# shinshoji01/Style-Restricted_GAN

Measured on AMD Instinct MI355X. Metric: images/sec G+D+E train step, CelebA 128x128 bs=32/GPU, higher is better.
Workload: dtype f32; 1 GPU; SRGAN-nopretrain (03-train) G+D+E train step, 128x128, bs=32/GPU, k=5, fp32, E trainable (BASELINE configs[1]); global_batch=32, unrolled_k=5, parallelism=dp1, graph_fallback=False, graph_segments=1, ranks_seen=1, execution=hipGraph replay of the captured step

## Files before the change

### style-restricted_gan_amd/csrc/conv_wino.hip

```cpp
#include <algorithm>
#include <cstdlib>
#include <type_traits>
#include "common.h"
#include "pack_device.h"

#ifndef WINO_EXP
#define WINO_EXP 0
#endif

namespace srgan {

constexpr int WT = 64;
constexpr int WNB = 64;
constexpr int WC = 8;

__device__ __forceinline__ auto uniform_rsrc(const float* base, unsigned bytes) {
  const unsigned long long a = reinterpret_cast<unsigned long long>(base);
  const unsigned lo = __builtin_amdgcn_readfirstlane((unsigned)a), hi = __builtin_amdgcn_readfirstlane((unsigned)(a >> 32));
  float* q = reinterpret_cast<float*>(((unsigned long long)hi << 32) | lo);
  return __builtin_amdgcn_make_buffer_rsrc(q, 0, __builtin_amdgcn_readfirstlane(bytes), 0x00020000);
}



template <int MODE, bool MASK = false>
__global__ __launch_bounds__(512) void wino_kernel(WinoParams p) {
  static_assert(!MASK || MODE == 2, "the mask epilogue exists for the transposed form only");
  constexpr int VH = 64 * 4 + 16, VP = 2 * VH + 32, VSZ = 16 * VP;
  static_assert(2 * VSZ <= 32768, "V buffers must fit the epilogue image");
  __shared__ __attribute__((aligned(16))) float lds[32768];
  __shared__ int tile_o[WT];
  __shared__ int tile_f[WT];
  constexpr int OT = MODE == 0 ? 2 : 3;
  constexpr int PS = MODE == 2 ? 2 : 1;
  const int ph_r = MODE == 2 ? (int)blockIdx.y >> 1 : 0, ph_s = MODE == 2 ? (int)blockIdx.y & 1 : 0;

  const int tid = threadIdx.x, lane = tid & 63, wave = tid >> 6;
  const int lr = lane & 31, lh = lane >> 5;
  int bid = blockIdx.x;
  const int nblk = gridDim.x;
  if ((nblk & 7) == 0) bid = (bid & 7) * (nblk >> 3) + (bid >> 3);
  const int m_tile = bid / p.n_tiles, n_tile = bid - m_tile * p.n_tiles;

  const int tl = tid >> 3, ch = tid & 7;
  constexpr unsigned kOutside = 0x80000000u;
  unsigned off[16];
  int g_b, g_ty, g_tx;
  bool g_tv;
  {
    const int t = m_tile * WT + tl;
    g_tv = t < p.T;
    const int tt = g_tv ? t : 0;
    const int per = p.TH * p.TW;
    g_b = tt / per;
    const int r = tt - g_b * per;
    g_ty = r / p.TW; g_tx = r - g_ty * p.TW;
    if (ch == 0) {
      const int oy = PS * OT * g_ty + ph_r, ox = PS * OT * g_tx + ph_s;
      const int nr = min(OT, (p.Ho - oy + PS - 1) / PS), nc = min(OT, (p.Wo - ox + PS - 1) / PS);
      tile_o[tl] = (g_tv && nr > 0 && nc > 0) ? (g_b * p.Ho + oy) * p.Wo + ox : -1;
      tile_f[tl] = max(nr, 0) | (max(nc, 0) << 4);
    }
  }
  auto set_offsets = [&](int phase) __attribute__((always_inline)) {
    int sy, dy_, oy0, ox0;
    if (MODE == 0) { sy = 2; dy_ = 1; oy0 = -p.pad; ox0 = -p.pad; }
    else if (MODE == 1) { sy = 6; dy_ = 2; oy0 = (phase >> 1) - p.pad; ox0 = (phase & 1) - p.pad; }
    else { sy = 3; dy_ = 1; oy0 = ph_r - 1; ox0 = ph_s - 1; }
#pragma unroll
    for (int i = 0; i < 4; ++i) {
      int iy = sy * g_ty + dy_ * i + oy0;
      bool yok = g_tv;
      if (MODE == 0 && p.reflect) {
        iy = iy < 0 ? -iy : iy;
        iy = iy >= p.H ? 2 * p.H - 2 - iy : iy;
        iy = min(max(iy, 0), p.H - 1);
      } else {
        yok = yok && (unsigned)iy < (unsigned)p.H;
      }
#pragma unroll
      for (int j = 0; j < 4; ++j) {
        int ix = sy * g_tx + dy_ * j + ox0;
        bool ok = yok;
        if (MODE == 0 && p.reflect) {
          ix = ix < 0 ? -ix : ix;
          ix = ix >= p.W ? 2 * p.W - 2 - ix : ix;
          ix = min(max(ix, 0), p.W - 1);
        } else {
          ok = ok && (unsigned)ix < (unsigned)p.W;
        }
        off[i * 4 + j] = ok ? (unsigned)(((g_b * p.H + iy) * p.W + ix) * p.C + ch) * 4u : kOutside;
      }
    }
  };
  set_offsets(0);
  const unsigned src_bytes = (unsigned)((size_t)p.NB * p.H * p.W * p.C * 4);
  const auto rs_x = uniform_rsrc(p.src, src_bytes);
  const auto rs_u = uniform_rsrc(p.u + ((size_t)(MODE == 2 ? blockIdx.y : 0) * p.n_tiles + n_tile) * p.nchunk * 8192,
                                 (unsigned)p.nchunk * 32768u);
  const unsigned ubase = (unsigned)((2 * wave) * 512 + lh * 256 + lr * 4) * 4u;

  float d[16];
  f32x4 bfr[2][2][2];
  int lc8 = 0, lphase = 0;
  auto load_x_part = [&](auto part_c) __attribute__((always_inline)) {
    constexpr int PART = decltype(part_c)::value;
#if WINO_EXP == 5 || WINO_EXP == 6
    if (lc8 + lphase > 0) return;
#endif
#pragma unroll
    for (int i = 4 * PART; i < 4 * PART + 4; ++i)
      d[i] = __builtin_bit_cast(float, __builtin_amdgcn_raw_buffer_load_b32(rs_x, off[i], lc8 * (WC * 4), 0));
    if constexpr (PART == 3) {
      ++lc8;
      if (MODE == 1 && lc8 == p.cpp) {
        lc8 = 0;
        ++lphase;
        set_offsets(lphase);
      }
    }
  };
  auto load_x = [&]() __attribute__((always_inline)) {
    load_x_part(std::integral_constant<int, 0>{});
    load_x_part(std::integral_constant<int, 1>{});
    load_x_part(std::integral_constant<int, 2>{});
    load_x_part(std::integral_constant<int, 3>{});
  };
  auto load_u1 = [&](int kc, auto par, int a, int j) __attribute__((always_inline)) {
    constexpr int P = decltype(par)::value;
#if WINO_EXP == 7
    if (kc > 1) return;
#endif
    bfr[P][a][j] = __builtin_bit_cast(f32x4, __builtin_amdgcn_raw_buffer_load_b128(rs_u, ubase + a * 2048 + j * 512, kc * 32768, 0));
  };
  auto load_u = [&](int kc, auto par) __attribute__((always_inline)) {
#pragma unroll
    for (int a = 0; a < 2; ++a)
#pragma unroll
      for (int j = 0; j < 2; ++j) load_u1(kc, par, a, j);
  };
  float tv[16];
  auto store_piece = [&](int buf, auto piece_c) __attribute__((always_inline)) {
    constexpr int PIECE = decltype(piece_c)::value;
#if WINO_EXP == 4 || WINO_EXP == 6
    return;
#endif
    float* V = lds + buf * VSZ + (ch >> 2) * VH + tl * 4 + (ch & 3);
    if constexpr (PIECE == 0) {
#if WINO_EXP == 9
      return;
#endif
#pragma unroll
      for (int c = 0; c < 4; ++c) {
        tv[0 * 4 + c] = d[0 * 4 + c] - d[2 * 4 + c];
        tv[1 * 4 + c] = d[1 * 4 + c] + d[2 * 4 + c];
        tv[2 * 4 + c] = d[2 * 4 + c] - d[1 * 4 + c];
        tv[3 * 4 + c] = d[1 * 4 + c] - d[3 * 4 + c];
      }
    } else {
#if WINO_EXP == 8
#pragma unroll
      for (int r = 2 * (PIECE - 1); r < 2 * PIECE; ++r) {
        asm volatile("" ::"v"(tv[r * 4 + 0] - tv[r * 4 + 2]), "v"(tv[r * 4 + 1] + tv[r * 4 + 2]), "v"(tv[r * 4 + 2] - tv[r * 4 + 1]),
                     "v"(tv[r * 4 + 1] - tv[r * 4 + 3]));
      }
      (void)V;
#elif WINO_EXP == 9
#pragma unroll
      for (int r = 2 * (PIECE - 1); r < 2 * PIECE; ++r) {
        V[(r * 4 + 0) * VP] = d[r * 4 + 0];
        V[(r * 4 + 1) * VP] = d[r * 4 + 1];
        V[(r * 4 + 2) * VP] = d[r * 4 + 2];
        V[(r * 4 + 3) * VP] = d[r * 4 + 3];
      }
#else
#pragma unroll
      for (int r = 2 * (PIECE - 1); r < 2 * PIECE; ++r) {
        V[(r * 4 + 0) * VP] = tv[r * 4 + 0] - tv[r * 4 + 2];
        V[(r * 4 + 1) * VP] = tv[r * 4 + 1] + tv[r * 4 + 2];
        V[(r * 4 + 2) * VP] = tv[r * 4 + 2] - tv[r * 4 + 1];
        V[(r * 4 + 3) * VP] = tv[r * 4 + 1] - tv[r * 4 + 3];
      }
#endif
    }
  };
  auto store_v = [&](int buf) __attribute__((always_inline)) {
    store_piece(buf, std::integral_constant<int, 0>{});
    store_piece(buf, std::integral_constant<int, 1>{});
    store_piece(buf, std::integral_constant<int, 2>{});
  };

  f32x16 acc[2][2][2];
#pragma unroll
  for (int a = 0; a < 2; ++a)
#pragma unroll
    for (int i = 0; i < 2; ++i)
#pragma unroll
      for (int j = 0; j < 2; ++j)
#pragma unroll
        for (int e = 0; e < 16; ++e) acc[a][i][j][e] = 0.f;

  f32x4 af[2][2];
  auto read_frags = [&](int buf, int slot) __attribute__((always_inline)) {
    const float* V = lds + buf * VSZ + (2 * wave + slot) * VP + lh * VH;
#pragma unroll
    for (int i = 0; i < 2; ++i) af[slot][i] = *reinterpret_cast<const f32x4*>(V + (i * 32 + lr) * 4);
  };
  auto mfma_steps = [&](auto par, int slot, int e0, int e1) __attribute__((always_inline)) {
    constexpr int P = decltype(par)::value;
#pragma unroll
    for (int e = e0; e < e1; ++e)
#pragma unroll
      for (int i = 0; i < 2; ++i)
#pragma unroll
        for (int j = 0; j < 2; ++j)
          acc[slot][i][j] = __builtin_amdgcn_mfma_f32_32x32x2f32(af[slot][i][e], bfr[P][slot][j][e], acc[slot][i][j], 0, 0, 0);
  };

  using I0 = std::integral_constant<int, 0>;
  using I1 = std::integral_constant<int, 1>;
  using I2 = std::integral_constant<int, 2>;
  using I3 = std::integral_constant<int, 3>;
  using T = std::true_type;
  using F = std::false_type;
  const int nk = p.nchunk;
  load_x();
  load_u(0, I0{});
  store_v(0);
  __syncthreads();
  read_frags(0, 0);
  if (nk > 1) load_x();
  auto iter = [&](int kc, auto par, auto st, auto ld) __attribute__((always_inline)) {
    constexpr bool ST = decltype(st)::value, LD = decltype(ld)::value;
    constexpr int P = decltype(par)::value;
    using NP = std::integral_constant<int, 1 - P>;
    auto sb = [&]() __attribute__((always_inline)) { __builtin_amdgcn_sched_barrier(0); };
    read_frags(P, 1);
    mfma_steps(par, 0, 0, 1);
    if constexpr (ST) store_piece(1 - P, I0{});
    sb();
    mfma_steps(par, 0, 1, 2);
    if constexpr (ST) store_piece(1 - P, I1{});
    if constexpr (LD) load_x_part(I0{});
    sb();
    mfma_steps(par, 0, 2, 3);
    if constexpr (ST) store_piece(1 - P, I2{});
    if constexpr (LD) load_x_part(I1{});
    sb();
    mfma_steps(par, 0, 3, 4);
    if constexpr (ST) load_u1(kc + 1, NP{}, 0, 0);
    if constexpr (LD) load_x_part(I2{});
    sb();
    mfma_steps(par, 1, 0, 1);
    if constexpr (ST) load_u1(kc + 1, NP{}, 0, 1);
    if constexpr (LD) load_x_part(I3{});
    sb();
    mfma_steps(par, 1, 1, 2);
    if constexpr (ST) { load_u1(kc + 1, NP{}, 1, 0); load_u1(kc + 1, NP{}, 1, 1); }
    sb();
    mfma_steps(par, 1, 2, 3);
    sb();
    __syncthreads();
    if constexpr (ST) read_frags(1 - P, 0);
    mfma_steps(par, 1, 3, 4);
  };
  {
    int kc = 0;
    for (; kc + 3 < nk; kc += 2) {
      iter(kc, I0{}, T{}, T{});
      iter(kc + 1, I1{}, T{}, T{});
    }
    iter(kc, I0{}, T{}, F{});
    iter(kc + 1, I1{}, F{}, F{});
  }

  const int cq = tid & 7, et = tid >> 3;
#pragma unroll
  for (int half = 0; half < 2; ++half) {
    __syncthreads();
#pragma unroll
    for (int a = 0; a < 2; ++a)
#pragma unroll
      for (int i = 0; i < 2; ++i)
#pragma unroll
        for (int e = 0; e < 16; ++e) {
          const int tile = i * 32 + (e & 3) + 8 * (e >> 2) + 4 * lh;
          lds[(2 * wave + a) * 2048 + tile * 32 + lr] = acc[a][i][half][e];
        }
    __syncthreads();
    const int n = n_tile * WNB + half * 32 + cq * 4;
    const bool nok = n < p.Cd;
    f32x4 bv = {0.f, 0.f, 0.f, 0.f};
    if (nok && p.bias) bv = *reinterpret_cast<const f32x4*>(p.bias + n);
    const int o = tile_o[et], f = tile_f[et];
    f32x4 mk[OT][OT];
    if constexpr (MASK) {
      if (nok && o >= 0) {
        const float* mp = p.mask + (size_t)o * p.Cd + n;
#pragma unroll
        for (int a = 0; a < OT; ++a)
#pragma unroll
          for (int b2 = 0; b2 < OT; ++b2)
            if (a < (f & 15) && b2 < (f >> 4)) mk[a][b2] = *reinterpret_cast<const f32x4*>(mp + (size_t)(a * p.Wo + b2) * PS * p.Cd);
      }
    }
    f32x4 m[16];
#pragma unroll
    for (int k = 0; k < 16; ++k) m[k] = *reinterpret_cast<const f32x4*>(lds + k * 2048 + et * 32 + cq * 4);
    f32x4 y[OT][OT];
    if constexpr (MODE == 0) {
      f32x4 s0[4], s1[4];
#pragma unroll
      for (int c = 0; c < 4; ++c) {
        s0[c] = m[0 * 4 + c] + m[1 * 4 + c] + m[2 * 4 + c];
        s1[c] = m[1 * 4 + c] - m[2 * 4 + c] - m[3 * 4 + c];
      }
      y[0][0] = s0[0] + s0[1] + s0[2]; y[0][1] = s0[1] - s0[2] - s0[3];
      y[1][0] = s1[0] + s1[1] + s1[2]; y[1][1] = s1[1] - s1[2] - s1[3];
    } else {
      f32x4 h[3][4];
#pragma unroll
      for (int c = 0; c < 4; ++c) {
        h[0][c] = m[0 * 4 + c] + 0.5f * (m[1 * 4 + c] + m[2 * 4 + c]);
        h[1][c] = 0.5f * (m[1 * 4 + c] - m[2 * 4 + c]);
        h[2][c] = 0.5f * (m[1 * 4 + c] + m[2 * 4 + c]) + m[3 * 4 + c];
      }
#pragma unroll
      for (int a = 0; a < 3; ++a) {
        y[a][0] = h[a][0] + 0.5f * (h[a][1] + h[a][2]);
        y[a][1] = 0.5f * (h[a][1] - h[a][2]);
        y[a][2] = 0.5f * (h[a][1] + h[a][2]) + h[a][3];
      }
    }
    if (nok && o >= 0) {
      const int nr = f & 15, nc = f >> 4;
      float* dp = p.dst + (size_t)o * p.Cd + n;
#pragma unroll
      for (int a = 0; a < OT; ++a)
#pragma unroll
        for (int b2 = 0; b2 < OT; ++b2)
          if (a < nr && b2 < nc) {
            f32x4 v = y[a][b2] + bv;
#pragma unroll
            for (int c = 0; c < 4; ++c) v[c] = apply_act(v[c], p.act, p.slope);
            if constexpr (MASK) {
#pragma unroll
              for (int c = 0; c < 4; ++c) v[c] *= act_grad(mk[a][b2][c], SRGAN_ACT_LRELU, p.mask_slope);
            }
            *reinterpret_cast<f32x4*>(dp + (size_t)(a * p.Wo + b2) * PS * p.Cd) = v;
          }
    }
  }
}

struct WinoWgradParams {
  const float* x;
  const float* dy;
  float* slab;
  int NB, H, W, C, Ho, Wo, O;
  int pad, reflect;
  int TH, TW;
  int groups;
  int groups_per_split, splits;
  int bsplits, nb_per;
  int o_tiles, i_tiles, Opad;
  int xcd_splits;
};

template <int MODE>
__global__ __launch_bounds__(512) void wino_wgrad_kernel(WinoWgradParams p) {
  __shared__ __attribute__((aligned(16))) float lds[32768];
  const int tid = threadIdx.x, lane = tid & 63, wave = tid >> 6;
  const int lr = lane & 31, lh = lane >> 5;
  int bid = blockIdx.x;
  const int tiles_per_split = p.o_tiles * p.i_tiles;
  int split;
  if (p.xcd_splits) {
    const int grp = bid / (8 * tiles_per_split), r = bid - grp * 8 * tiles_per_split;
    split = grp * 8 + (r & 7);
    bid = r >> 3;
  } else {
    split = bid / tiles_per_split;
    bid -= split * tiles_per_split;
  }
  const int o_tile = bid / p.i_tiles, i_tile = bid - o_tile * p.i_tiles;

  const int th = wave >> 2, tq = lane & 3;
  const int chl = (wave & 3) * 16 + (lane >> 2);
  constexpr int ND = MODE == 0 ? 4 : 9;
  constexpr int OT = MODE == 0 ? 2 : 3;
  const int phase = MODE == 1 ? (i_tile * 64) / p.C : 0;
  const int ph_p = phase >> 1, ph_q = phase & 1;
  const int ci = i_tile * 64 - phase * p.C + chl, co = o_tile * 64 + chl;
  constexpr unsigned kOutside = 0x80000000u;
  unsigned offx[16], offd[ND];
  auto set_group = [&](int g) __attribute__((always_inline)) {
    const int q = g * 8 + th * 4 + tq;
    const bool tv = q < p.TH * p.TW && g < p.groups;
    const int qq = tv ? q : 0;
    const int ty = qq / p.TW, tx = qq - ty * p.TW;
    const int sy = MODE == 0 ? 2 : 6, dstep = MODE == 0 ? 1 : 2;
    const int oy0 = (MODE == 0 ? 0 : ph_p) - p.pad, ox0 = (MODE == 0 ? 0 : ph_q) - p.pad;
#pragma unroll
    for (int i = 0; i < 4; ++i) {
      int iy = sy * ty + dstep * i + oy0;
      bool yok = tv && ci < p.C;
      if (p.reflect) {
        iy = iy < 0 ? -iy : iy;
        iy = iy >= p.H ? 2 * p.H - 2 - iy : iy;
        iy = min(max(iy, 0), p.H - 1);
      } else {
        yok = yok && (unsigned)iy < (unsigned)p.H;
      }
#pragma unroll
      for (int j = 0; j < 4; ++j) {
        int ix = sy * tx + dstep * j + ox0;
        bool ok = yok;
        if (p.reflect) {
          ix = ix < 0 ? -ix : ix;
          ix = ix >= p.W ? 2 * p.W - 2 - ix : ix;
          ix = min(max(ix, 0), p.W - 1);
        } else {
          ok = ok && (unsigned)ix < (unsigned)p.W;
        }
        offx[i * 4 + j] = ok ? (unsigned)((iy * p.W + ix) * p.C + ci) * 4u : kOutside;
      }
    }
#pragma unroll
    for (int i = 0; i < OT; ++i)
#pragma unroll
      for (int j = 0; j < OT; ++j) {
        const int oy = OT * ty + i, ox = OT * tx + j;
        const bool ok = tv && co < p.O && oy < p.Ho && ox < p.Wo;
        offd[i * OT + j] = ok ? (unsigned)((oy * p.Wo + ox) * p.O + co) * 4u : kOutside;
      }
  };
  const unsigned x_img = (unsigned)(p.H * p.W * p.C) * 4u, d_img = (unsigned)(p.Ho * p.Wo * p.O) * 4u;
  const auto rs_x = uniform_rsrc(p.x, x_img * (unsigned)p.NB);
  const auto rs_d = uniform_rsrc(p.dy, d_img * (unsigned)p.NB);

  const int gsplit = split / p.bsplits, bsplit = split - gsplit * p.bsplits;
  const int g0 = gsplit * p.groups_per_split;
  const int g1 = min(g0 + p.groups_per_split, p.groups);
  const int b0 = bsplit * p.nb_per, b1 = min(b0 + p.nb_per, p.NB);
  const int nk = max(g1 - g0, 0) * max(b1 - b0, 0);
  int lg = g0, lb = b0;
  set_group(lg);
  float dx[16], dd[ND];
  auto load_part = [&](auto part_c) __attribute__((always_inline)) {
    constexpr int PART = decltype(part_c)::value;
    if constexpr (PART < 4) {
#pragma unroll
      for (int i = 4 * PART; i < 4 * PART + 4; ++i)
        dx[i] = __builtin_bit_cast(float, __builtin_amdgcn_raw_buffer_load_b32(rs_x, offx[i], lb * x_img, 0));
    } else {
#pragma unroll
      for (int i = 0; i < ND; ++i)
        dd[i] = __builtin_bit_cast(float, __builtin_amdgcn_raw_buffer_load_b32(rs_d, offd[i], lb * d_img, 0));
      if (++lb == b1) {
        lb = b0;
        ++lg;
        set_group(lg);
      }
    }
  };
  auto load_chunk = [&]() __attribute__((always_inline)) {
    load_part(std::integral_constant<int, 0>{});
    load_part(std::integral_constant<int, 1>{});
    load_part(std::integral_constant<int, 2>{});
    load_part(std::integral_constant<int, 3>{});
    load_part(std::integral_constant<int, 4>{});
  };
  const int wofs = th * 256 + (wave & 3) * 64 + lane;
  float tv[16];
  auto store_piece = [&](int buf, auto piece_c) __attribute__((always_inline)) {
    constexpr int PIECE = decltype(piece_c)::value;
    float* Z = lds + buf * 16384 + wofs;
    float* V = Z + 8192;
    if constexpr (PIECE == 0) {
#pragma unroll
      for (int c = 0; c < 4; ++c) {
        tv[0 * 4 + c] = dx[0 * 4 + c] - dx[2 * 4 + c];
        tv[1 * 4 + c] = dx[1 * 4 + c] + dx[2 * 4 + c];
        tv[2 * 4 + c] = dx[2 * 4 + c] - dx[1 * 4 + c];
        tv[3 * 4 + c] = dx[1 * 4 + c] - dx[3 * 4 + c];
      }
    } else if constexpr (PIECE == 1 || PIECE == 2) {
#pragma unroll
      for (int r = 2 * (PIECE - 1); r < 2 * PIECE; ++r) {
        V[(r * 4 + 0) * 512] = tv[r * 4 + 0] - tv[r * 4 + 2];
        V[(r * 4 + 1) * 512] = tv[r * 4 + 1] + tv[r * 4 + 2];
        V[(r * 4 + 2) * 512] = tv[r * 4 + 2] - tv[r * 4 + 1];
        V[(r * 4 + 3) * 512] = tv[r * 4 + 1] - tv[r * 4 + 3];
      }
    } else if constexpr (MODE == 0) {
      const float r0[2] = {dd[0], dd[1]};
      const float r1[2] = {dd[0] + dd[2], dd[1] + dd[3]};
      const float r2[2] = {dd[0] - dd[2], dd[1] - dd[3]};
      const float r3[2] = {-dd[2], -dd[3]};
      const float* rr[4] = {r0, r1, r2, r3};
#pragma unroll
      for (int r = 0; r < 4; ++r) {
        Z[(r * 4 + 0) * 512] = rr[r][0];
        Z[(r * 4 + 1) * 512] = rr[r][0] + rr[r][1];
        Z[(r * 4 + 2) * 512] = rr[r][0] - rr[r][1];
        Z[(r * 4 + 3) * 512] = -rr[r][1];
      }
    } else {
      float zr[4][3];
#pragma unroll
      for (int l = 0; l < 3; ++l) {
        zr[0][l] = dd[0 * 3 + l];
        zr[1][l] = 0.5f * (dd[0 * 3 + l] + dd[1 * 3 + l] + dd[2 * 3 + l]);
        zr[2][l] = 0.5f * (dd[0 * 3 + l] - dd[1 * 3 + l] + dd[2 * 3 + l]);
        zr[3][l] = dd[2 * 3 + l];
      }
#pragma unroll
      for (int r = 0; r < 4; ++r) {
        Z[(r * 4 + 0) * 512] = zr[r][0];
        Z[(r * 4 + 1) * 512] = 0.5f * (zr[r][0] + zr[r][1] + zr[r][2]);
        Z[(r * 4 + 2) * 512] = 0.5f * (zr[r][0] - zr[r][1] + zr[r][2]);
        Z[(r * 4 + 3) * 512] = zr[r][2];
      }
    }
  };
  auto store_chunk = [&](int buf) __attribute__((always_inline)) {
    store_piece(buf, std::integral_constant<int, 0>{});
    store_piece(buf, std::integral_constant<int, 1>{});
    store_piece(buf, std::integral_constant<int, 2>{});
    store_piece(buf, std::integral_constant<int, 3>{});
  };

  f32x16 acc[2][2][2];
#pragma unroll
  for (int a = 0; a < 2; ++a)
#pragma unroll
    for (int i = 0; i < 2; ++i)
#pragma unroll
      for (int j = 0; j < 2; ++j)
#pragma unroll
        for (int e = 0; e < 16; ++e) acc[a][i][j][e] = 0.f;
  f32x4 af[2][2], bf[2][2];
  auto read_frags = [&](int buf, int slot) __attribute__((always_inline)) {
    const float* Z = lds + buf * 16384 + (2 * wave + slot) * 512 + lh * 256;
    const float* V = Z + 8192;
#pragma unroll
    for (int i = 0; i < 2; ++i) af[slot][i] = *reinterpret_cast<const f32x4*>(Z + (i * 32 + lr) * 4);
#pragma unroll
    for (int j = 0; j < 2; ++j) bf[slot][j] = *reinterpret_cast<const f32x4*>(V + (j * 32 + lr) * 4);
  };
  auto mfma_steps = [&](int slot, int e0, int e1) __attribute__((always_inline)) {
#pragma unroll
    for (int e = e0; e < e1; ++e)
#pragma unroll
      for (int i = 0; i < 2; ++i)
#pragma unroll
        for (int j = 0; j < 2; ++j)
          acc[slot][i][j] = __builtin_amdgcn_mfma_f32_32x32x2f32(af[slot][i][e], bf[slot][j][e], acc[slot][i][j], 0, 0, 0);
  };

  using T = std::true_type;
  using F = std::false_type;
  if (nk > 0) {
    load_chunk();
    store_chunk(0);
    __syncthreads();
    read_frags(0, 0);
    if (nk > 1) load_chunk();
    auto iter = [&](int kc, auto st, auto ld) __attribute__((always_inline)) {
      constexpr bool ST = decltype(st)::value, LD = decltype(ld)::value;
      const int cur = kc & 1;
      auto sb = [&]() __attribute__((always_inline)) { __builtin_amdgcn_sched_barrier(0); };
      read_frags(cur, 1);
      mfma_steps(0, 0, 1);
      if constexpr (ST) store_piece(cur ^ 1, std::integral_constant<int, 0>{});
      sb();
      mfma_steps(0, 1, 2);
      if constexpr (ST) store_piece(cur ^ 1, std::integral_constant<int, 1>{});
      if constexpr (LD) load_part(std::integral_constant<int, 0>{});
      sb();
      mfma_steps(0, 2, 3);
      if constexpr (ST) store_piece(cur ^ 1, std::integral_constant<int, 2>{});
      if constexpr (LD) load_part(std::integral_constant<int, 1>{});
      sb();
      mfma_steps(0, 3, 4);
      if constexpr (ST) store_piece(cur ^ 1, std::integral_constant<int, 3>{});
      if constexpr (LD) load_part(std::integral_constant<int, 2>{});
      sb();
      mfma_steps(1, 0, 1);
      if constexpr (LD) load_part(std::integral_constant<int, 3>{});
      sb();
      mfma_steps(1, 1, 2);
      if constexpr (LD) load_part(std::integral_constant<int, 4>{});
      sb();
      mfma_steps(1, 2, 3);
      sb();
      __syncthreads();
      if constexpr (ST) read_frags(cur ^ 1, 0);
      mfma_steps(1, 3, 4);
    };
    int kc = 0;
    for (; kc + 2 < nk; ++kc) iter(kc, T{}, T{});
    if (nk >= 2) iter(nk - 2, T{}, F{});
    iter(nk - 1, F{}, F{});
  }

  const int cq = tid & 7, row = tid >> 3;
  constexpr int NT = MODE == 0 ? 9 : 16;
  float* slab = p.slab + (size_t)split * p.Opad * (NT * p.C);
#pragma unroll
  for (int half = 0; half < 2; ++half) {
    __syncthreads();
#pragma unroll
    for (int a = 0; a < 2; ++a)
#pragma unroll
      for (int i = 0; i < 2; ++i)
#pragma unroll
        for (int e = 0; e < 16; ++e) {
          const int r = i * 32 + (e & 3) + 8 * (e >> 2) + 4 * lh;
          lds[(2 * wave + a) * 2048 + r * 32 + lr] = acc[a][i][half][e];
        }
    __syncthreads();
    const int ic = i_tile * 64 - phase * p.C + half * 32 + cq * 4;
    const int oc = o_tile * 64 + row;
    f32x4 u[16];
#pragma unroll
    for (int k = 0; k < 16; ++k) u[k] = *reinterpret_cast<const f32x4*>(lds + k * 2048 + row * 32 + cq * 4);
    if (oc < p.O && ic < p.C) {
      float* dst = slab + (size_t)oc * (NT * p.C) + ic;
      if constexpr (MODE == 0) {
        f32x4 h[3][4];
#pragma unroll
        for (int c = 0; c < 4; ++c) {
          h[0][c] = u[0 * 4 + c] + 0.5f * (u[1 * 4 + c] + u[2 * 4 + c]);
          h[1][c] = 0.5f * (u[1 * 4 + c] - u[2 * 4 + c]);
          h[2][c] = 0.5f * (u[1 * 4 + c] + u[2 * 4 + c]) + u[3 * 4 + c];
        }
#pragma unroll
        for (int a = 0; a < 3; ++a) {
          *reinterpret_cast<f32x4*>(dst + (a * 3 + 0) * p.C) = h[a][0] + 0.5f * (h[a][1] + h[a][2]);
          *reinterpret_cast<f32x4*>(dst + (a * 3 + 1) * p.C) = 0.5f * (h[a][1] - h[a][2]);
          *reinterpret_cast<f32x4*>(dst + (a * 3 + 2) * p.C) = 0.5f * (h[a][1] + h[a][2]) + h[a][3];
        }
      } else {
        f32x4 h[2][4];
#pragma unroll
        for (int c = 0; c < 4; ++c) {
          h[0][c] = u[0 * 4 + c] + u[1 * 4 + c] + u[2 * 4 + c];
          h[1][c] = u[1 * 4 + c] - u[2 * 4 + c] - u[3 * 4 + c];
        }
#pragma unroll
        for (int a = 0; a < 2; ++a) {
          const int ky = 2 * a + ph_p;
          *reinterpret_cast<f32x4*>(dst + (ky * 4 + 0 + ph_q) * p.C) = h[a][0] + h[a][1] + h[a][2];
          *reinterpret_cast<f32x4*>(dst + (ky * 4 + 2 + ph_q) * p.C) = h[a][1] - h[a][2] - h[a][3];
        }
      }
    }
  }
}

__global__ __launch_bounds__(256) void wino_pack_kernel(WinoPackParams p) {
  const long long total = wino_pack_total(p);
  if (wino43_pack_block_ok(p)) {
    __shared__ float tile[32 * WP43_ROW];
    for (long long base = (long long)blockIdx.x * 256; base < total; base += (long long)gridDim.x * 256)
      wino43_pack_block(p, base, tile);
    return;
  }
  for (long long idx = (long long)blockIdx.x * blockDim.x + threadIdx.x; idx < total;
       idx += (long long)gridDim.x * blockDim.x)
    wino_pack_item(p, idx);
}

static double conv_flops_of(const srgan_conv_desc* d) {
  return 2.0 * d->N * d->Ho * d->Wo * (double)d->O * d->kh * d->kw * d->I;
}

static bool wino_disabled() {
  static const bool off = SRGAN_AB_SET("SRGAN_NO_WINOGRAD");
  return off;
}
double wino_threshold_scale() {
  const char* e = std::getenv("SRGAN_WINOGRAD_THRESHOLD_SCALE");
  return e ? std::atof(e) : 1.0;
}
static bool wino43_disabled() {
  static const bool off = SRGAN_AB_SET("SRGAN_NO_WINOGRAD43");
  return off;
}
static bool wino_s2_disabled() {
  static const bool off = SRGAN_AB_SET("SRGAN_NO_WINOGRAD_S2");
  return off;
}
static bool wino42_disabled() {
  static const bool off = SRGAN_AB_SET("SRGAN_NO_WINOGRAD42");
  return off;
}

static int wino_variant(const srgan_conv_desc* d, int kind) {
  if (compute_bf16()) {
    if (halo16_applicable(d, kind)) return 4;
    if (kind == 1 && halo16t_applicable(d)) return 5;
    return kind == 0 && halo16s_applicable(d) ? 6 : 0;
  }
  if (wino_disabled()) return 0;

  const int C = kind == 0 ? d->I : d->O, N = kind == 0 ? d->O : d->I;
  if (C % (2 * WC) != 0 || C < 32 || N < 32 || N % 4 != 0) return 0;
  const long long src_elems = (long long)d->N * (kind == 0 ? (long long)d->Hi * d->Wi * d->I : (long long)d->Ho * d->Wo * d->O);
  if (src_elems >= (1LL << 29)) return 0;
  if (d->kh == 3 && d->kw == 3 && d->stride == 1 && d->pad == 1) {
    if (d->Hi < 3 || d->Wi < 3) return 0;
    const int ho = kind == 0 ? d->Ho : d->Hi, wo = kind == 0 ? d->Wo : d->Wi;
    if (!wino43_disabled() && d->pad_mode == SRGAN_PAD_ZERO && ho % 4 == 0 && wo % 4 == 0 && N % 32 == 0 && C % 32 == 0) {
      const long long b43 = ceil_div((long long)d->N * (ho / 4) * (wo / 4), 64) * (N / 32);
      if (b43 >= 50 * wino_threshold_scale()) return 3;
    }
    const long long blocks = ceil_div((long long)d->N * ceil_div(ho, 2) * ceil_div(wo, 2), WT) * ceil_div(N, WNB);
    return blocks >= 100 * wino_threshold_scale() ? 1 : 0;
  }
  if (d->kh == 4 && d->kw == 4 && d->stride == 2 && d->pad == 1 && d->pad_mode == SRGAN_PAD_ZERO && !wino_s2_disabled()) {
    if ((d->Hi & 1) || (d->Wi & 1)) return 0;
    const long long dst_elems = (long long)d->N * (kind == 0 ? (long long)d->Ho * d->Wo * d->O : (long long)d->Hi * d->Wi * d->I);
    if (!wino42_disabled() && d->Ho % 4 == 0 && d->Wo % 4 == 0 && N % 64 == 0 && C % 16 == 0 && dst_elems < (1LL << 30) &&
        (kind == 1 || C <= 128)) {
      const long long b42 = ceil_div((long long)d->N * (d->Ho / 4) * (d->Wo / 4), 32) * (N / 64) * (kind == 1 ? 4 : 1);
      if (b42 >= 120 * wino_threshold_scale()) return 7;
    }
    const long long th = ceil_div(d->Ho, 3), tw = ceil_div(d->Wo, 3);
    const double eff = (double)d->Ho * d->Wo / (9.0 * th * tw);
    if (eff * 2.25 < 1.5) return 0;
    const long long blocks = ceil_div((long long)d->N * th * tw, WT) * ceil_div(N, WNB) * (kind == 1 ? 4 : 1);
    return blocks >= 120 * wino_threshold_scale() ? 2 : 0;
  }
  return 0;
}

bool wino_applicable(const srgan_conv_desc* d, int kind) { return wino_variant(d, kind) != 0; }

static void wino_dims(const srgan_conv_desc* d, int kind, int* C, int* N, int* n_tiles, int* nchunk, int* phases) {
  const int v = wino_variant(d, kind);
  *C = kind == 0 ? d->I : d->O;
  *N = kind == 0 ? d->O : d->I;
  *n_tiles = v == 7 ? *N / 64 : (v >= 4) ? 1 : v == 3 ? *N / 32 : (int)ceil_div(*N, WNB);
  *nchunk = v == 7 ? (kind == 0 ? 4 : 1) * (*C / 16) : (v >= 4) ? *C / 32 : (v == 2 && kind == 0 ? 4 : 1) * (*C / WC);
  *phases = ((v == 2 || v == 7) && kind == 1) ? 4 : 1;
}

size_t wino_packed_bytes(const srgan_conv_desc* d, int kind) {
  int C, N, n_tiles, nchunk, phases;
  wino_dims(d, kind, &C, &N, &n_tiles, &nchunk, &phases);
  if (wino_variant(d, kind) == 4) return halo16_packed_bytes(d);
  if (wino_variant(d, kind) == 6) return halo16s_packed_bytes(d);
  if (wino_variant(d, kind) == 5) return halo16t_packed_bytes(d);
  if (wino_variant(d, kind) == 3) return (size_t)n_tiles * nchunk * (36 * 256) * sizeof(float);
  if (wino_variant(d, kind) == 7) return (size_t)phases * n_tiles * nchunk * (25 * 1024) * sizeof(float);
  return (size_t)phases * n_tiles * nchunk * 8192 * sizeof(float);
}

size_t wino_scratch_bytes(const srgan_conv_desc* d, int kind) {
  if (wino_variant(d, kind) != 3) return 0;
  const int ho = kind == 0 ? d->Ho : d->Hi, wo = kind == 0 ? d->Wo : d->Wi;
  return wino43_scratch_floats((long long)d->N * (ho / 4) * (wo / 4), kind == 0 ? d->I : d->O) * sizeof(float);
}

bool wino43_wgrad_geometry(const srgan_conv_desc* d, Wino43WgradGeom* g) {
  static const bool off = SRGAN_AB_SET("SRGAN_NO_WINOGRAD43_WGRAD");
  if (off || wino_variant(d, 0) != 3 || d->I % 64 != 0 || d->O % 32 != 0) return false;
  const long long T = (long long)d->N * (d->Ho / 4) * (d->Wo / 4);
  const long long ntc = ceil_div(T, 64) * 8;
  const int tiles = (d->O / 32) * (d->I / 64);
  long long splits = std::max(1, 256 / tiles);
  long long cps = std::max<long long>(2, ceil_div(ntc, splits));
  if (ntc % cps == 1) ++cps;
  splits = ceil_div(ntc, cps);
  if (ntc < 2 || ntc - (splits - 1) * cps < 2) return false;
  g->NB = d->N; g->H = d->Ho; g->W = d->Wo; g->C = d->I; g->O = d->O; g->ntc = (int)ntc;
  g->splits = (int)splits; g->chunks_per_split = (int)cps;
  g->v_bytes = wino_scratch_bytes(d, 0);
  g->z_bytes = (size_t)(d->O / 32) * ntc * 36 * 256 * sizeof(float);
  g->slab_bytes = (size_t)splits * d->O * 9 * d->I * sizeof(float);
  return g->v_bytes < (1ULL << 32) && g->z_bytes < (1ULL << 32);
}

void wino_pack_params(const srgan_conv_desc* d, int kind, const float* w, float* dst, WinoPackParams* out) {
  WinoPackParams q{};
  int C, N;
  wino_dims(d, kind, &C, &N, &q.n_tiles, &q.nchunk, &q.phases);
  q.variant = wino_variant(d, kind);
  q.w = w; q.dst = dst; q.sO = d->sO; q.sI = d->sI; q.sH = d->sH; q.sW = d->sW; q.N = N; q.C = C; q.kind = kind;
  q.no_block = std::getenv("SRGAN_PACK_ITEM_PATH") != nullptr ? 1 : 0;
  *out = q;
}

int wino_pack(const srgan_conv_desc* d, int kind, const float* w, float* dst, hipStream_t st) {
  WinoPackParams q{};
  wino_pack_params(d, kind, w, dst, &q);
  const long long total = wino_pack_total(q);
  hipLaunchKernelGGL(wino_pack_kernel, dim3((unsigned)std::min<long long>(ceil_div(total, 256), 4096)), dim3(256), 0, st, q);
  return check_launch("wino_pack_kernel");
}

bool wino43_fwd_applicable(const srgan_conv_desc* d) { return wino_variant(d, 0) == 3; }
bool wino43_dgrad_applicable(const srgan_conv_desc* d) { return d->pad_mode == SRGAN_PAD_ZERO && wino_variant(d, 1) == 3; }

int wino_run(const srgan_conv_desc* d, int kind, const float* src, const float* packed, const float* bias, float* dst,
             int act, float slope, float* scratch, hipStream_t st, const float* res, bool* res_done, bool v_ready,
             const float* mask, float mask_slope, bool* mask_done) {
  if (res_done) *res_done = false;
  if (mask_done) *mask_done = false;
  WinoParams p{};
  p.act = act; p.slope = slope;
  int C, N, phases;
  wino_dims(d, kind, &C, &N, &p.n_tiles, &p.nchunk, &phases);
  const int variant = wino_variant(d, kind);
  SRGAN_REQUIRE(variant != 0, "winograd: layer not applicable");
  if (variant == 6) {
    SRGAN_REQUIRE(!v_ready && !res && !mask, "halo16s: no prepared image, skip tensor or mask on this path");
    return halo16s_run(d, src, packed, bias, dst, act, slope, conv_flops_of(d), st);
  }
  if (variant == 5) {
    SRGAN_REQUIRE(!v_ready && !bias && act == SRGAN_ACT_NONE, "halo16t: plain transposed product only");
    return halo16t_run(d, src, packed, dst, conv_flops_of(d), st);
  }
  if (variant == 4) {
    SRGAN_REQUIRE(!v_ready, "halo16: no transformed-input image on this path");
    if (res_done) *res_done = res != nullptr;
    return halo16_run(d, kind, src, packed, bias, res, dst, act, slope, conv_flops_of(d), st);
  }
  const bool reflect = d->pad_mode == SRGAN_PAD_REFLECT;
  p.src = src; p.u = packed; p.bias = bias; p.dst = dst;
  p.NB = d->N; p.C = C; p.Cd = N; p.cpp = C / WC;
  int ot = 2;
  if (variant == 1 || variant == 3) {
    if (kind == 0) {
      p.H = d->Hi; p.W = d->Wi; p.Ho = d->Ho; p.Wo = d->Wo; p.pad = d->pad; p.reflect = reflect ? 1 : 0;
    } else {
      p.H = d->Ho; p.W = d->Wo; p.reflect = 0;
      p.pad = reflect ? 2 : 2 - d->pad;
      p.Ho = d->Ho + 2 * p.pad - 2; p.Wo = d->Wo + 2 * p.pad - 2;
    }
    if (variant == 3) { ot = 4; p.TH = p.Ho / 4; p.TW = p.Wo / 4; }
    else { p.TH = (p.Ho + 1) / 2; p.TW = (p.Wo + 1) / 2; }
  } else {
    ot = variant == 7 ? 4 : 3;
    p.pad = d->pad; p.reflect = 0;
    if (kind == 0) { p.H = d->Hi; p.W = d->Wi; p.Ho = d->Ho; p.Wo = d->Wo; }
    else { p.H = d->Ho; p.W = d->Wo; p.Ho = d->Hi; p.Wo = d->Wi; }
    p.TH = (int)ceil_div(d->Ho, ot); p.TW = (int)ceil_div(d->Wo, ot);
    if (variant == 7) p.cpp = C / 16;
  }
  (void)ot;
  const long long T = (long long)p.NB * p.TH * p.TW;
  SRGAN_REQUIRE(T < (1LL << 30), "winograd: too many tiles");
  p.T = (int)T;
  p.m_tiles = (int)ceil_div(T, variant == 7 ? 32 : WT);
  const long long grid = (long long)p.m_tiles * p.n_tiles;
  SRGAN_REQUIRE(grid < (1LL << 31), "winograd: grid too large");
  if (variant == 3) {
    SRGAN_REQUIRE(p.pad == 1 && p.Ho == p.H && p.Wo == p.W && p.nchunk >= 2 && p.Cd % 32 == 0 && p.C % 32 == 0,
                  "winograd F(4,3): geometry");
    SRGAN_REQUIRE(scratch, "winograd F(4,3): no scratch for the transformed input");
    p.res = res;
    if (res_done) *res_done = res != nullptr;
    wino43_launch(p, scratch, grid, conv_flops_of(d), st, v_ready);
    return check_launch("wino43_kernel");
  }
  SRGAN_REQUIRE(!v_ready, "winograd: a prepared V image only serves the F(4x4,3x3) path");
  if (variant == 7) {
    SRGAN_REQUIRE(p.pad == 1 && p.nchunk >= 2 && p.Cd % 64 == 0 && p.C % 16 == 0 && d->Ho % 4 == 0 && d->Wo % 4 == 0, "winograd F(4,2): geometry");
    if (kind == 1 && mask) {
      p.mask = mask; p.mask_slope = mask_slope;
      if (mask_done) *mask_done = true;
    }
    return wino42_launch(p, kind, grid, kind == 1 && mask != nullptr, conv_flops_of(d), st);
  }
  ProfToken tok = prof_begin(variant == 1 ? 14 : 16, conv_flops_of(d), st);
  if (variant == 1) hipLaunchKernelGGL(wino_kernel<0>, dim3((unsigned)grid), dim3(512), 0, st, p);
  else if (kind == 0) hipLaunchKernelGGL(wino_kernel<1>, dim3((unsigned)grid), dim3(512), 0, st, p);
  else if (mask) {
    p.mask = mask; p.mask_slope = mask_slope;
    if (mask_done) *mask_done = true;
    hipLaunchKernelGGL((wino_kernel<2, true>), dim3((unsigned)grid, 4), dim3(512), 0, st, p);
  } else hipLaunchKernelGGL(wino_kernel<2>, dim3((unsigned)grid, 4), dim3(512), 0, st, p);
  prof_end(tok, st);
  return check_launch("wino_kernel");
}

static int wino_wgrad_geometry(const srgan_conv_desc* d, WinoWgradParams* p) {
  static const bool off = SRGAN_AB_SET("SRGAN_NO_WINOGRAD_WGRAD");
  if (wino_disabled() || off || compute_bf16()) return 0;
  int variant = 0;
  if (d->kh == 3 && d->kw == 3 && d->stride == 1 && d->pad == 1) variant = 1;
  else if (d->kh == 4 && d->kw == 4 && d->stride == 2 && d->pad == 1 && d->pad_mode == SRGAN_PAD_ZERO && !(d->Hi & 1) &&
           !(d->Wi & 1) && !wino_s2_disabled())
    variant = 2;
  if (variant == 0) return 0;
  if (d->I % 64 != 0 || d->O % 64 != 0 || d->Hi < 3 || d->Wi < 3) return 0;
  if ((long long)d->N * d->Hi * d->Wi * d->I >= (1LL << 29) || (long long)d->N * d->Ho * d->Wo * d->O >= (1LL << 29)) return 0;
  const int ot = variant == 1 ? 2 : 3;
  p->NB = d->N; p->H = d->Hi; p->W = d->Wi; p->C = d->I; p->Ho = d->Ho; p->Wo = d->Wo; p->O = d->O;
  p->pad = d->pad; p->reflect = d->pad_mode == SRGAN_PAD_REFLECT ? 1 : 0;
  p->TH = (int)ceil_div(d->Ho, ot); p->TW = (int)ceil_div(d->Wo, ot);
  if (variant == 2 && (double)d->Ho * d->Wo / ((double)ot * ot * p->TH * p->TW) * 2.25 < 1.5) return 0;
  p->groups = (int)ceil_div((long long)p->TH * p->TW, 8);
  if (variant == 2 && (double)d->Ho * d->Wo / ((double)ot * ot * 8 * p->groups) * 2.25 < 1.5) return 0;
  p->o_tiles = d->O / 64; p->i_tiles = (variant == 2 ? 4 : 1) * d->I / 64; p->Opad = d->O;
  const int tiles = p->o_tiles * p->i_tiles;
  int splits = std::max(1, 256 / tiles);
  splits = std::min(splits, p->groups);
  p->groups_per_split = (int)ceil_div(p->groups, splits);
  p->splits = (int)ceil_div(p->groups, p->groups_per_split);
  p->bsplits = 1; p->nb_per = d->N;
  long long blocks = (long long)tiles * p->splits, chunks = (long long)p->groups_per_split * d->N;
  const double ts = wino_threshold_scale();
  static const int min_chunks_b = SRGAN_AB_INT("SRGAN_WGRAD_BSPLIT_MIN_CHUNKS", 24);
  if (variant == 2 && min_chunks_b > 0 && blocks < 192) {
    const int S = std::max(1, 256 / tiles);
    long long best_blocks = blocks, best_chunks = chunks;
    int best_gps = p->groups_per_split, best_gs = p->splits, best_bs = 1, best_nb = d->N;
    for (int gs = 1; gs <= std::min(p->groups, S); ++gs) {
      const int gps = (int)ceil_div(p->groups, gs), gse = (int)ceil_div(p->groups, gps);
      const int bs = std::max(1, std::min(d->N, S / gse));
      const int nb = (int)ceil_div(d->N, bs), bse = (int)ceil_div(d->N, nb);
      const long long bl = (long long)tiles * gse * bse, ch = (long long)gps * nb;
      if (ch < min_chunks_b) continue;
      if (bl > best_blocks || (bl == best_blocks && (ch > best_chunks || (ch == best_chunks && nb > best_nb)))) {
        best_blocks = bl; best_chunks = ch; best_gps = gps; best_gs = gse; best_bs = bse; best_nb = nb;
      }
    }
    if (best_bs > 1) {
      p->groups_per_split = best_gps; p->bsplits = best_bs; p->nb_per = best_nb;
      p->splits = best_gs * best_bs;
      blocks = best_blocks; chunks = best_chunks;
    }
  }
  if (variant == 1) {
    if (blocks < 16 * ts || chunks < 4 * ts) return 0;
  } else {
    static const int min_blocks = SRGAN_AB_INT("SRGAN_WGRAD_S2_MIN_BLOCKS", 192);
    if (blocks < min_blocks * ts || chunks < (p->bsplits > 1 ? min_chunks_b : 48) * ts) return 0;
  }
  return variant;
}

bool wino_wgrad_applicable(const srgan_conv_desc* d) {
  if (compute_bf16()) return halo16_wgrad_applicable(d);
  WinoWgradParams p{};
  return wino_wgrad_geometry(d, &p) != 0;
}

void wino_wgrad_slab(const srgan_conv_desc* d, int* splits, int* Cdpad, int* NNpad) {
  if (compute_bf16()) { halo16_wgrad_slab(d, splits, Cdpad, NNpad); return; }
  WinoWgradParams p{};
  wino_wgrad_geometry(d, &p);
  *splits = p.splits; *Cdpad = p.Opad; *NNpad = d->kh * d->kw * d->I;
}

int wino_wgrad_run(const srgan_conv_desc* d, const float* x, const float* dy, float* slab, hipStream_t st) {
  if (compute_bf16()) return halo16_wgrad_run(d, x, dy, slab, conv_flops_of(d), st);
  WinoWgradParams p{};
  const int variant = wino_wgrad_geometry(d, &p);
  SRGAN_REQUIRE(variant != 0, "winograd wgrad: layer not applicable");
  p.x = x; p.dy = dy; p.slab = slab;
  p.xcd_splits = (p.splits % 8 == 0) ? 1 : 0;
  ProfToken tok = prof_begin(variant == 1 ? 15 : 17, conv_flops_of(d), st);
  const dim3 grid((unsigned)(p.o_tiles * p.i_tiles * p.splits));
  if (variant == 1) hipLaunchKernelGGL(wino_wgrad_kernel<0>, grid, dim3(512), 0, st, p);
  else hipLaunchKernelGGL(wino_wgrad_kernel<1>, grid, dim3(512), 0, st, p);
  prof_end(tok, st);
  return check_launch("wino_wgrad_kernel");
}

}
```

Before: 527.3 images/sec.

## Make F(2x2,3x3) winograd kernel persistent with cross-tile prefetch

The MODE 0 winograd forward kernel becomes persistent. The grid is capped at the CU count, and each block walks a contiguous range of output tiles. While the current tile's main loop and epilogue run, the next tile's input offsets are decoded, its first chunk is loaded and its V pieces are stored, so prologue latency overlaps the previous tile. The tile metadata arrays are double-buffered, and the U buffer resource now covers all n_tiles. This adds sync points and register pressure, and capping the grid can cut parallelism and unbalance the tail.

```diff
diff --git a/style-restricted_gan_amd/csrc/conv_wino.hip b/style-restricted_gan_amd/csrc/conv_wino.hip
--- a/style-restricted_gan_amd/csrc/conv_wino.hip
+++ b/style-restricted_gan_amd/csrc/conv_wino.hip
@@ -26,11 +26,12 @@
 template <int MODE, bool MASK = false>
 __global__ __launch_bounds__(512) void wino_kernel(WinoParams p) {
   static_assert(!MASK || MODE == 2, "the mask epilogue exists for the transposed form only");
+  constexpr bool PERSIST = MODE == 0;
   constexpr int VH = 64 * 4 + 16, VP = 2 * VH + 32, VSZ = 16 * VP;
   static_assert(2 * VSZ <= 32768, "V buffers must fit the epilogue image");
   __shared__ __attribute__((aligned(16))) float lds[32768];
-  __shared__ int tile_o[WT];
-  __shared__ int tile_f[WT];
+  __shared__ int tile_o[PERSIST ? 2 : 1][WT];
+  __shared__ int tile_f[PERSIST ? 2 : 1][WT];
   constexpr int OT = MODE == 0 ? 2 : 3;
   constexpr int PS = MODE == 2 ? 2 : 1;
   const int ph_r = MODE == 2 ? (int)blockIdx.y >> 1 : 0, ph_s = MODE == 2 ? (int)blockIdx.y & 1 : 0;
@@ -40,14 +41,23 @@
   int bid = blockIdx.x;
   const int nblk = gridDim.x;
   if ((nblk & 7) == 0) bid = (bid & 7) * (nblk >> 3) + (bid >> 3);
-  const int m_tile = bid / p.n_tiles, n_tile = bid - m_tile * p.n_tiles;
+  int item = bid, item_end = bid + 1;
+  if constexpr (PERSIST) {
+    const int n_items = p.m_tiles * p.n_tiles;
+    const int q = n_items / nblk, r = n_items - q * nblk;
+    item = bid * q + min(bid, r);
+    item_end = item + q + (bid < r ? 1 : 0);
+  }
 
   const int tl = tid >> 3, ch = tid & 7;
   constexpr unsigned kOutside = 0x80000000u;
   unsigned off[16];
   int g_b, g_ty, g_tx;
   bool g_tv;
-  {
+  int ld_n_tile = 0;
+  auto decode_item = [&](int it, int par) __attribute__((always_inline)) {
+    const int m_tile = it / p.n_tiles;
+    ld_n_tile = it - m_tile * p.n_tiles;
     const int t = m_tile * WT + tl;
     g_tv = t < p.T;
     const int tt = g_tv ? t : 0;
@@ -58,10 +68,11 @@
     if (ch == 0) {
       const int oy = PS * OT * g_ty + ph_r, ox = PS * OT * g_tx + ph_s;
       const int nr = min(OT, (p.Ho - oy + PS - 1) / PS), nc = min(OT, (p.Wo - ox + PS - 1) / PS);
-      tile_o[tl] = (g_tv && nr > 0 && nc > 0) ? (g_b * p.Ho + oy) * p.Wo + ox : -1;
-      tile_f[tl] = max(nr, 0) | (max(nc, 0) << 4);
-    }
-  }
+      tile_o[par][tl] = (g_tv && nr > 0 && nc > 0) ? (g_b * p.Ho + oy) * p.Wo + ox : -1;
+      tile_f[par][tl] = max(nr, 0) | (max(nc, 0) << 4);
+    }
+  };
+  decode_item(item, 0);
   auto set_offsets = [&](int phase) __attribute__((always_inline)) {
     int sy, dy_, oy0, ox0;
     if (MODE == 0) { sy = 2; dy_ = 1; oy0 = -p.pad; ox0 = -p.pad; }
@@ -96,8 +107,8 @@
   set_offsets(0);
   const unsigned src_bytes = (unsigned)((size_t)p.NB * p.H * p.W * p.C * 4);
   const auto rs_x = uniform_rsrc(p.src, src_bytes);
-  const auto rs_u = uniform_rsrc(p.u + ((size_t)(MODE == 2 ? blockIdx.y : 0) * p.n_tiles + n_tile) * p.nchunk * 8192,
-                                 (unsigned)p.nchunk * 32768u);
+  const auto rs_u = uniform_rsrc(p.u + (size_t)(MODE == 2 ? blockIdx.y : 0) * p.n_tiles * p.nchunk * 8192,
+                                 (unsigned)(p.n_tiles * p.nchunk) * 32768u);
   const unsigned ubase = (unsigned)((2 * wave) * 512 + lh * 256 + lr * 4) * 4u;
 
   float d[16];
@@ -191,14 +202,6 @@
   };
 
   f32x16 acc[2][2][2];
-#pragma unroll
-  for (int a = 0; a < 2; ++a)
-#pragma unroll
-    for (int i = 0; i < 2; ++i)
-#pragma unroll
-      for (int j = 0; j < 2; ++j)
-#pragma unroll
-        for (int e = 0; e < 16; ++e) acc[a][i][j][e] = 0.f;
 
   f32x4 af[2][2];
   auto read_frags = [&](int buf, int slot) __attribute__((always_inline)) {
@@ -224,132 +227,169 @@
   using T = std::true_type;
   using F = std::false_type;
   const int nk = p.nchunk;
+  int n_tile = ld_n_tile;
+  int ipar = 0;
   load_x();
-  load_u(0, I0{});
+  load_u(n_tile * nk, I0{});
   store_v(0);
   __syncthreads();
   read_frags(0, 0);
   if (nk > 1) load_x();
-  auto iter = [&](int kc, auto par, auto st, auto ld) __attribute__((always_inline)) {
+  auto iter = [&](int un, auto par, auto st, auto ld, auto tail) __attribute__((always_inline)) {
     constexpr bool ST = decltype(st)::value, LD = decltype(ld)::value;
+    constexpr bool NEXT = decltype(tail)::value == 1, LAST = decltype(tail)::value == 2;
     constexpr int P = decltype(par)::value;
     using NP = std::integral_constant<int, 1 - P>;
     auto sb = [&]() __attribute__((always_inline)) { __builtin_amdgcn_sched_barrier(0); };
     read_frags(P, 1);
     mfma_steps(par, 0, 0, 1);
     if constexpr (ST) store_piece(1 - P, I0{});
+    if constexpr (NEXT) {
+      if (item + 1 < item_end) {
+        decode_item(item + 1, ipar ^ 1);
+        set_offsets(0);
+      } else {
+#pragma unroll
+        for (int i = 0; i < 16; ++i) off[i] = kOutside;
+      }
+      lc8 = 0;
+    }
     sb();
     mfma_steps(par, 0, 1, 2);
-    if constexpr (ST) store_piece(1 - P, I1{});
+    if constexpr (ST && !LAST) store_piece(1 - P, I1{});
     if constexpr (LD) load_x_part(I0{});
     sb();
     mfma_steps(par, 0, 2, 3);
-    if constexpr (ST) store_piece(1 - P, I2{});
+    if constexpr (ST && !LAST) store_piece(1 - P, I2{});
     if constexpr (LD) load_x_part(I1{});
     sb();
     mfma_steps(par, 0, 3, 4);
-    if constexpr (ST) load_u1(kc + 1, NP{}, 0, 0);
+    if constexpr (ST) load_u1(un, NP{}, 0, 0);
     if constexpr (LD) load_x_part(I2{});
     sb();
     mfma_steps(par, 1, 0, 1);
-    if constexpr (ST) load_u1(kc + 1, NP{}, 0, 1);
+    if constexpr (ST) load_u1(un, NP{}, 0, 1);
     if constexpr (LD) load_x_part(I3{});
     sb();
     mfma_steps(par, 1, 1, 2);
-    if constexpr (ST) { load_u1(kc + 1, NP{}, 1, 0); load_u1(kc + 1, NP{}, 1, 1); }
+    if constexpr (ST) { load_u1(un, NP{}, 1, 0); load_u1(un, NP{}, 1, 1); }
     sb();
     mfma_steps(par, 1, 2, 3);
     sb();
     __syncthreads();
-    if constexpr (ST) read_frags(1 - P, 0);
+    if constexpr (ST && !LAST) read_frags(1 - P, 0);
     mfma_steps(par, 1, 3, 4);
   };
-  {
+  for (;;) {
+#pragma unroll
+    for (int a = 0; a < 2; ++a)
+#pragma unroll
+      for (int i = 0; i < 2; ++i)
+#pragma unroll
+        for (int j = 0; j < 2; ++j)
+#pragma unroll
+          for (int e = 0; e < 16; ++e) acc[a][i][j][e] = 0.f;
+    const int u0 = n_tile * nk;
     int kc = 0;
     for (; kc + 3 < nk; kc += 2) {
-      iter(kc, I0{}, T{}, T{});
-      iter(kc + 1, I1{}, T{}, T{});
-    }
-    iter(kc, I0{}, T{}, F{});
-    iter(kc + 1, I1{}, F{}, F{});
-  }
-
-  const int cq = tid & 7, et = tid >> 3;
-#pragma unroll
-  for (int half = 0; half < 2; ++half) {
+      iter(u0 + kc + 1, I0{}, T{}, T{}, I0{});
+      iter(u0 + kc + 2, I1{}, T{}, T{}, I0{});
+    }
+    if constexpr (PERSIST) {
+      iter(u0 + kc + 1, I0{}, T{}, T{}, I1{});
+      iter(ld_n_tile * nk, I1{}, T{}, T{}, I2{});
+    } else {
+      iter(u0 + kc + 1, I0{}, T{}, F{}, I0{});
+      iter(0, I1{}, F{}, F{}, I0{});
+    }
+
+    const int cq = tid & 7, et = tid >> 3;
+#pragma unroll
+    for (int half = 0; half < 2; ++half) {
+      __syncthreads();
+#pragma unroll
+      for (int a = 0; a < 2; ++a)
+#pragma unroll
+        for (int i = 0; i < 2; ++i)
+#pragma unroll
+          for (int e = 0; e < 16; ++e) {
+            const int tile = i * 32 + (e & 3) + 8 * (e >> 2) + 4 * lh;
+            lds[(2 * wave + a) * 2048 + tile * 32 + lr] = acc[a][i][half][e];
+          }
+      __syncthreads();
+      const int n = n_tile * WNB + half * 32 + cq * 4;
+      const bool nok = n < p.Cd;
+      f32x4 bv = {0.f, 0.f, 0.f, 0.f};
+      if (nok && p.bias) bv = *reinterpret_cast<const f32x4*>(p.bias + n);
+      const int o = tile_o[ipar][et], f = tile_f[ipar][et];
+      f32x4 mk[OT][OT];
+      if constexpr (MASK) {
+        if (nok && o >= 0) {
+          const float* mp = p.mask + (size_t)o * p.Cd + n;
+#pragma unroll
+          for (int a = 0; a < OT; ++a)
+#pragma unroll
+            for (int b2 = 0; b2 < OT; ++b2)
+              if (a < (f & 15) && b2 < (f >> 4)) mk[a][b2] = *reinterpret_cast<const f32x4*>(mp + (size_t)(a * p.Wo + b2) * PS * p.Cd);
+        }
+      }
+      f32x4 m[16];
+#pragma unroll
+      for (int k = 0; k < 16; ++k) m[k] = *reinterpret_cast<const f32x4*>(lds + k * 2048 + et * 32 + cq * 4);
+      if (PERSIST && half == 1 && item + 1 < item_end) {
+        __syncthreads();
+        store_piece(0, I1{});
+        store_piece(0, I2{});
+      }
+      f32x4 y[OT][OT];
+      if constexpr (MODE == 0) {
+        f32x4 s0[4], s1[4];
+#pragma unroll
+        for (int c = 0; c < 4; ++c) {
+          s0[c] = m[0 * 4 + c] + m[1 * 4 + c] + m[2 * 4 + c];
+          s1[c] = m[1 * 4 + c] - m[2 * 4 + c] - m[3 * 4 + c];
+        }
+        y[0][0] = s0[0] + s0[1] + s0[2]; y[0][1] = s0[1] - s0[2] - s0[3];
+        y[1][0] = s1[0] + s1[1] + s1[2]; y[1][1] = s1[1] - s1[2] - s1[3];
+      } else {
+        f32x4 h[3][4];
+#pragma unroll
+        for (int c = 0; c < 4; ++c) {
+          h[0][c] = m[0 * 4 + c] + 0.5f * (m[1 * 4 + c] + m[2 * 4 + c]);
+          h[1][c] = 0.5f * (m[1 * 4 + c] - m[2 * 4 + c]);
+          h[2][c] = 0.5f * (m[1 * 4 + c] + m[2 * 4 + c]) + m[3 * 4 + c];
+        }
+#pragma unroll
+        for (int a = 0; a < 3; ++a) {
+          y[a][0] = h[a][0] + 0.5f * (h[a][1] + h[a][2]);
+          y[a][1] = 0.5f * (h[a][1] - h[a][2]);
+          y[a][2] = 0.5f * (h[a][1] + h[a][2]) + h[a][3];
+        }
+      }
+      if (nok && o >= 0) {
+        const int nr = f & 15, nc = f >> 4;
+        float* dp = p.dst + (size_t)o * p.Cd + n;
+#pragma unroll
+        for (int a = 0; a < OT; ++a)
+#pragma unroll
+          for (int b2 = 0; b2 < OT; ++b2)
+            if (a < nr && b2 < nc) {
+              f32x4 v = y[a][b2] + bv;
+#pragma unroll
+              for (int c = 0; c < 4; ++c) v[c] = apply_act(v[c], p.act, p.slope);
+              if constexpr (MASK) {
+#pragma unroll
+                for (int c = 0; c < 4; ++c) v[c] *= act_grad(mk[a][b2][c], SRGAN_ACT_LRELU, p.mask_slope);
+              }
+              *reinterpret_cast<f32x4*>(dp + (size_t)(a * p.Wo + b2) * PS * p.Cd) = v;
+            }
+      }
+    }
+    if (!PERSIST || ++item >= item_end) break;
+    n_tile = ld_n_tile;
+    ipar ^= 1;
     __syncthreads();
-#pragma unroll
-    for (int a = 0; a < 2; ++a)
-#pragma unroll
-      for (int i = 0; i < 2; ++i)
-#pragma unroll
-        for (int e = 0; e < 16; ++e) {
-          const int tile = i * 32 + (e & 3) + 8 * (e >> 2) + 4 * lh;
-          lds[(2 * wave + a) * 2048 + tile * 32 + lr] = acc[a][i][half][e];
-        }
-    __syncthreads();
-    const int n = n_tile * WNB + half * 32 + cq * 4;
-    const bool nok = n < p.Cd;
-    f32x4 bv = {0.f, 0.f, 0.f, 0.f};
-    if (nok && p.bias) bv = *reinterpret_cast<const f32x4*>(p.bias + n);
-    const int o = tile_o[et], f = tile_f[et];
-    f32x4 mk[OT][OT];
-    if constexpr (MASK) {
-      if (nok && o >= 0) {
-        const float* mp = p.mask + (size_t)o * p.Cd + n;
-#pragma unroll
-        for (int a = 0; a < OT; ++a)
-#pragma unroll
-          for (int b2 = 0; b2 < OT; ++b2)
-            if (a < (f & 15) && b2 < (f >> 4)) mk[a][b2] = *reinterpret_cast<const f32x4*>(mp + (size_t)(a * p.Wo + b2) * PS * p.Cd);
-      }
-    }
-    f32x4 m[16];
-#pragma unroll
-    for (int k = 0; k < 16; ++k) m[k] = *reinterpret_cast<const f32x4*>(lds + k * 2048 + et * 32 + cq * 4);
-    f32x4 y[OT][OT];
-    if constexpr (MODE == 0) {
-      f32x4 s0[4], s1[4];
-#pragma unroll
-      for (int c = 0; c < 4; ++c) {
-        s0[c] = m[0 * 4 + c] + m[1 * 4 + c] + m[2 * 4 + c];
-        s1[c] = m[1 * 4 + c] - m[2 * 4 + c] - m[3 * 4 + c];
-      }
-      y[0][0] = s0[0] + s0[1] + s0[2]; y[0][1] = s0[1] - s0[2] - s0[3];
-      y[1][0] = s1[0] + s1[1] + s1[2]; y[1][1] = s1[1] - s1[2] - s1[3];
-    } else {
-      f32x4 h[3][4];
-#pragma unroll
-      for (int c = 0; c < 4; ++c) {
-        h[0][c] = m[0 * 4 + c] + 0.5f * (m[1 * 4 + c] + m[2 * 4 + c]);
-        h[1][c] = 0.5f * (m[1 * 4 + c] - m[2 * 4 + c]);
-        h[2][c] = 0.5f * (m[1 * 4 + c] + m[2 * 4 + c]) + m[3 * 4 + c];
-      }
-#pragma unroll
-      for (int a = 0; a < 3; ++a) {
-        y[a][0] = h[a][0] + 0.5f * (h[a][1] + h[a][2]);
-        y[a][1] = 0.5f * (h[a][1] - h[a][2]);
-        y[a][2] = 0.5f * (h[a][1] + h[a][2]) + h[a][3];
-      }
-    }
-    if (nok && o >= 0) {
-      const int nr = f & 15, nc = f >> 4;
-      float* dp = p.dst + (size_t)o * p.Cd + n;
-#pragma unroll
-      for (int a = 0; a < OT; ++a)
-#pragma unroll
-        for (int b2 = 0; b2 < OT; ++b2)
-          if (a < nr && b2 < nc) {
-            f32x4 v = y[a][b2] + bv;
-#pragma unroll
-            for (int c = 0; c < 4; ++c) v[c] = apply_act(v[c], p.act, p.slope);
-            if constexpr (MASK) {
-#pragma unroll
-              for (int c = 0; c < 4; ++c) v[c] *= act_grad(mk[a][b2][c], SRGAN_ACT_LRELU, p.mask_slope);
-            }
-            *reinterpret_cast<f32x4*>(dp + (size_t)(a * p.Wo + b2) * PS * p.Cd) = v;
-          }
-    }
+    read_frags(0, 0);
   }
 }
 
@@ -876,8 +916,14 @@
     }
     return wino42_launch(p, kind, grid, kind == 1 && mask != nullptr, conv_flops_of(d), st);
   }
+  static const int cus = [] {
+    int dev = 0, n = 0;
+    (void)hipGetDevice(&dev);
+    (void)hipDeviceGetAttribute(&n, hipDeviceAttributeMultiprocessorCount, dev);
+    return n > 0 ? n : 256;
+  }();
   ProfToken tok = prof_begin(variant == 1 ? 14 : 16, conv_flops_of(d), st);
-  if (variant == 1) hipLaunchKernelGGL(wino_kernel<0>, dim3((unsigned)grid), dim3(512), 0, st, p);
+  if (variant == 1) hipLaunchKernelGGL(wino_kernel<0>, dim3((unsigned)std::min<long long>(grid, cus)), dim3(512), 0, st, p);
   else if (kind == 0) hipLaunchKernelGGL(wino_kernel<1>, dim3((unsigned)grid), dim3(512), 0, st, p);
   else if (mask) {
     p.mask = mask; p.mask_slope = mask_slope;
```

After: 526.9 images/sec (median of 2 runs). About the same (-0.1%).
